# succinctlabs/kzg-rs

Hardware: AMD Instinct MI355X
Metric: blobs/sec verify_blob_kzg_proof_batch (higher is better)
Workload: dtype u32 limbs (255-bit Fr / 381-bit Fp modular integers); 1 GPU; verify_blob_kzg_proof_batch, batches of 1024 synthetic blobs (4096 Fr each), device-resident, known-tau test setup (BASELINE.json configs[1]); one step = one launch group of 256 independent batches = 262144 blobs per GPU; blobs_per_gpu_per_batch=1024, batch=1024, parallelism=shard-by-blob x1, groups_in_flight=4

## Files before the change

kzg_rs_amd/csrc/capi_settings.hpp:

```cpp

#include <atomic>
#include <condition_variable>
#include <deque>
#include <memory>
struct DevProgram {
    SlpProgram p{};
    void* blob = nullptr;
};

struct DevProgram2 {
    Slp2Program p{};
    void* blob = nullptr;
};

constexpr size_t MAX_WORLD = 64;
constexpr size_t LATENCY_PAIRING_MAX = 32;
constexpr size_t MAX_BATCHES_PER_LAUNCH = 16384;
constexpr unsigned MSM_MAX_SLICES = 32;
constexpr size_t SLICED_MAX_BLOBS = 16384;
constexpr size_t LATENCY_MAX_BLOBS = 4096;
struct Workspace {
    size_t cap_n = 0;
    size_t cap_b = 0;
    size_t pending_n = 0, pending_b = 0, finish_b = 0;
// ... 177 lines not shown
    return run_program(s->verify, d_in, s->d_prep, d_out, instances, st);
}

static KzgRet settings_build(KzgSettings* s, const uint8_t tau_g2[96]);
static KzgRet settings_common(KzgSettings** out, const uint8_t tau_g2[96]) {
    int ndev = 0;
    if (hipGetDeviceCount(&ndev) != hipSuccess || ndev == 0) {
        (void)hipGetLastError();
        return fail(KZG_ERROR, "no HIP device: this library has no CPU fallback");
    }
    KzgSettings* s = new KzgSettings();
    KzgRet rc = settings_build(s, tau_g2);
    if (rc != KZG_OK) {
        const std::string msg = g_err;
        kzg_settings_free(s);
        g_err = msg;
        return rc;
    }
    if (opt_flag("coalesce", true)) {
        s->small = new SmallQueue();
        s->small->max_lanes = (size_t)std::max(1L, std::min((long)SMALL_LANES_MAX, opt_int("small_lanes", 2)));
        s->small->lane_two_streams = ab_int("small_streams", 3) == 2;
        s->small->lane_priority = ab_int("small_priority", 1) ? 1 : 0;
        s->small->linger_us = std::max(0L, std::min(2000L, opt_int("small_linger_us", 250)));
        s->small->linger_gap_us = std::max(1L, std::min(1000L, ab_int("small_linger_gap_us", 40)));
        s->small->cap_proofs = (size_t)std::max(1L, std::min(1024L, ab_int("small_cap_proofs", 1024)));
    }
    *out = s;
    return KZG_OK;
}
static KzgRet stream_make(hipStream_t* st, int priority) {
    if (priority) {
        int least = 0, greatest = 0;
        HIPCHK(hipDeviceGetStreamPriorityRange(&least, &greatest));
        HIPCHK(hipStreamCreateWithPriority(st, hipStreamNonBlocking, greatest));
    } else HIPCHK(hipStreamCreateWithFlags(st, hipStreamNonBlocking));
    return KZG_OK;
}
static KzgRet settings_streams(KzgSettings* s, bool single_stream, int priority = 0) {
    HIPCHK(hipGetDevice(&s->device));
    s->stream_priority = priority;
    KzgRet rc_s = stream_make(&s->s_plain[0], priority);
    if (rc_s != KZG_OK) return rc_s;
    s->s1 = s->s_sha = s->s_plain[0];
    HIPCHK(hipDeviceGetAttribute(&s->n_cus, hipDeviceAttributeMultiprocessorCount, s->device));
    if (single_stream) s->s2 = s->s1;
    else {
        if ((rc_s = stream_make(&s->s_plain[1], priority)) != KZG_OK) return rc_s;
        s->s2 = s->s_plain[1];
    }
    for (auto& e : s->ev) HIPCHK(hipEventCreate(&e));
    return KZG_OK;
}
static KzgRet settings_lane(KzgSettings** out, const KzgSettings* parent, int priority = 0) {
    KzgSettings* l = new KzgSettings();
    l->borrowed = true;
    l->d_M = parent->d_M; l->d_DM = parent->d_DM; l->d_M29 = parent->d_M29; l->d_DM29 = parent->d_DM29;
    l->d_eval_a = parent->d_eval_a; l->d_eval_b = parent->d_eval_b; l->d_eval_c = parent->d_eval_c;
    l->d_tau4 = parent->d_tau4; l->d_prep = parent->d_prep; l->d_prep29 = parent->d_prep29;
    l->d_gen_mult = parent->d_gen_mult; l->d_gen_mult_aff = parent->d_gen_mult_aff;
    l->prep = parent->prep; l->verify = parent->verify; l->verify2 = parent->verify2;
    l->scalars = parent->scalars; l->verify3 = parent->verify3; l->d_fixed_base = parent->d_fixed_base;
    memcpy(l->tau_g2_bytes, parent->tau_g2_bytes, 96);
    KzgRet rc = settings_streams(l, !parent->s_plain[1], priority);
    if (rc != KZG_OK) {
        const std::string msg = g_err;
        kzg_settings_free(l);
        g_err = msg;
        return rc;
    }
    *out = l;
    return KZG_OK;
}
static KzgRet settings_build(KzgSettings* s, const uint8_t tau_g2[96]) {
    memcpy(s->tau_g2_bytes, tau_g2, 96);
    KzgRet rc_streams = settings_streams(s, opt_flag("single_stream", false));
    if (rc_streams != KZG_OK) return rc_streams;
    HIPCHK(hipMalloc(&s->d_M, sizeof(Fr) * FE_PER_BLOB));
    HIPCHK(hipMalloc(&s->d_DM, sizeof(Fr) * FE_PER_BLOB));
    HIPCHK(hipMalloc(&s->d_M29, sizeof(Fr29Mem) * FE_PER_BLOB));
    HIPCHK(hipMalloc(&s->d_DM29, sizeof(Fr29Mem) * FE_PER_BLOB));
    hipLaunchKernelGGL(k_roots_tables, dim3(FE_PER_BLOB / 64), dim3(64), 0, s->s1, s->d_M, s->d_DM);
    hipLaunchKernelGGL(k_roots_tables29, dim3(FE_PER_BLOB / 64), dim3(64), 0, s->s1, s->d_M, s->d_M29, s->d_DM29);
    HIPCHK(hipMalloc(&s->d_eval_a, sizeof(uint4) * EVAL_SLOTS * 64));
    HIPCHK(hipMalloc(&s->d_eval_b, sizeof(uint4) * EVAL_SLOTS * 64));
    HIPCHK(hipMalloc(&s->d_eval_c, 4 * EVAL_SLOTS * 64));
    hipLaunchKernelGGL(k_eval_tables, dim3(EVAL_SLOTS), dim3(64), 0, s->s1, s->d_M29, s->d_DM29, s->d_eval_a, s->d_eval_b, s->d_eval_c);
    HIPCHK(hipGetLastError());
    KzgRet rc;
    if ((rc = upload_program(s->prep, kzg_slp_prep_begin, kzg_slp_prep_end)) != KZG_OK) return rc;
    if ((rc = upload_program(s->verify, kzg_slp_verify_begin, kzg_slp_verify_end)) != KZG_OK) return rc;
    if ((rc = upload_program2(s->verify2, kzg_slp_verify2_begin, kzg_slp_verify2_end)) != KZG_OK) return rc;
    if ((rc = upload_program2(s->scalars, kzg_slp_scalars_begin, kzg_slp_scalars_end)) != KZG_OK) return rc;
    if ((rc = upload_program2(s->verify3, kzg_slp_verify3_begin, kzg_slp_verify3_end)) != KZG_OK) return rc;
    if ((size_t)(kzg_fixed_base_end - kzg_fixed_base_begin) != FB_TABLE_BYTES) return fail(KZG_ERROR, "embedded fixed-base table has the wrong size");
    HIPCHK(hipMalloc(&s->d_fixed_base, FB_TABLE_BYTES));
    HIPCHK(hipMemcpy(s->d_fixed_base, kzg_fixed_base_begin, FB_TABLE_BYTES, hipMemcpyHostToDevice));
    DevTmp t_bytes, t_flag, t_q;
    HIPCHK(hipMalloc(&t_bytes.p, 96));
    HIPCHK(hipMalloc(&t_flag.p, 4));
    HIPCHK(hipMalloc(&t_q.p, sizeof(Fp) * 8));
    uint8_t* d_bytes = t_bytes.as<uint8_t>();
    uint32_t* d_flag = t_flag.as<uint32_t>();
    Fp* d_q = t_q.as<Fp>();
    HIPCHK(hipMalloc(&s->d_tau4, sizeof(Fp) * 4));
    HIPCHK(hipMalloc(&s->d_prep, sizeof(Fp) * 2 * s->prep.p.n_out));
    HIPCHK(hipMemcpyAsync(d_bytes, tau_g2, 96, hipMemcpyHostToDevice, s->s1));
    hipLaunchKernelGGL(k_g2_decompress, dim3(1), dim3(64), 0, s->s1, d_bytes, d_q, d_flag);
    hipLaunchKernelGGL(k_g2_generator, dim3(1), dim3(64), 0, s->s1, d_q + 4);
    HIPCHK(hipGetLastError());
    uint32_t flag = 0;
    HIPCHK(hipMemcpyAsync(&flag, d_flag, 4, hipMemcpyDeviceToHost, s->s1));
    HIPCHK(hipMemcpyAsync(s->d_tau4, d_q, sizeof(Fp) * 4, hipMemcpyDeviceToDevice, s->s1));
    if ((rc = run_program(s->prep, d_q, nullptr, s->d_prep, 2, s->s1)) != KZG_OK) return rc;
    {
        const int np = (int)(2 * s->prep.p.n_out);
        HIPCHK(hipMalloc(&s->d_prep29, (size_t)64 * np));
        hipLaunchKernelGGL(k_fp_to_fp29mem, dim3((unsigned)((np + 63) / 64)), dim3(64), 0, s->s1, s->d_prep, s->d_prep29, np);
        HIPCHK(hipGetLastError());
    }
    {
        DevTmp t_g, t_gf, t_gm;
        HIPCHK(hipMalloc(&t_g.p, sizeof(G1Aff)));
        HIPCHK(hipMalloc(&t_gf.p, 4));
        constexpr int NG = MSM_CHUNKS + MSM_CHUNKS_LATENCY;
        HIPCHK(hipMalloc(&t_gm.p, sizeof(G1Jac) * NG));
        G1Aff* d_g = t_g.as<G1Aff>();
        uint32_t* d_gf = t_gf.as<uint32_t>();
        G1Jac* d_gm = t_gm.as<G1Jac>();
        hipLaunchKernelGGL(k_set_generator, dim3(1), dim3(64), 0, s->s1, d_g, d_gf, 0);
        hipLaunchKernelGGL(k_g1_multiples, dim3(1), dim3(64), 0, s->s1, d_g, d_gf, d_gm, 1, 1, MSM_CHUNKS);
        hipLaunchKernelGGL(k_g1_multiples, dim3(1), dim3(64), 0, s->s1, d_g, d_gf, d_gm + MSM_CHUNKS, 1, 1, MSM_CHUNKS_LATENCY);
        HIPCHK(hipMalloc(&s->d_gen_mult, sizeof(G1Jac29Mem) * NG));
        hipLaunchKernelGGL(k_jac_to_jac29, dim3(1), dim3(64), 0, s->s1, d_gm, (G1Jac29Mem*)s->d_gen_mult, NG);
        HIPCHK(hipMalloc(&s->d_gen_mult_aff, sizeof(G1Aff29Mem) * MSM_CHUNKS));
        hipLaunchKernelGGL(k_jac29_to_aff29, dim3(1), dim3(64), 0, s->s1, (const G1Jac29Mem*)s->d_gen_mult, s->d_gen_mult_aff, MSM_CHUNKS);
        HIPCHK(hipGetLastError());
        HIPCHK(hipStreamSynchronize(s->s1));
    }
    HIPCHK(hipStreamSynchronize(s->s1));
    if (flag != G1_OK) return fail(KZG_BAD_SETUP, "g2_points[1] is not a valid (finite) compressed G2 point");
    if (s->verify.p.n_set != 2 * s->prep.p.n_out || s->verify.p.n_in != 6 || s->prep.p.n_in != 4 || s->verify2.p.n_set != s->verify.p.n_set ||
        s->verify2.p.n_in != 6 || s->verify2.p.n_out != s->verify.p.n_out)
        return fail(KZG_ERROR, "embedded SLP programs do not fit together");
    if (s->scalars.p.n_in != (uint32_t)SCALARS_INPUTS || s->scalars.p.n_set != 0 || !s->scalars.p.out_values || s->scalars.p.n_out + 6 != (uint32_t)VERIFY3_INPUTS ||
        s->verify3.p.n_in != (uint32_t)VERIFY3_INPUTS || s->verify3.p.n_set != s->verify.p.n_set || s->verify3.p.n_out != (uint32_t)VERIFY3_OUTPUTS || s->verify3.p.out_values)
        return fail(KZG_ERROR, "embedded one-proof programs do not fit together");
    return KZG_OK;
}

static KzgRet settings_load_points(KzgSettings* s, const std::vector<uint8_t>& g1b, const std::vector<uint8_t>& g2b, int N, size_t n2) {
    DevTmp t_bytes, t_flag2, t_gflag, t_tmp;
    HIPCHK(hipMalloc(&t_bytes.p, std::max(g1b.size(), g2b.size())));
    HIPCHK(hipMalloc(&t_flag2.p, 4 * (size_t)N));
    HIPCHK(hipMalloc(&t_tmp.p, sizeof(G1Aff) * (size_t)N));
    uint8_t* d_bytes = t_bytes.as<uint8_t>();
    uint32_t* d_flag2 = t_flag2.as<uint32_t>();
    G1Aff* d_tmp = t_tmp.as<G1Aff>();
    HIPCHK(hipMalloc(&s->d_g1, sizeof(G1Aff) * (size_t)N));
    HIPCHK(hipMalloc(&s->d_g1_flag, 4 * (size_t)N));
    HIPCHK(hipMalloc(&s->d_g1_mult, MULT_ENTRY_BYTES * MSM_CHUNKS * (size_t)N));
    HIPCHK(hipMemcpyAsync(d_bytes, g1b.data(), g1b.size(), hipMemcpyHostToDevice, s->s1));
    hipLaunchKernelGGL(k_g1_decode, dim3((unsigned)((N + 63) / 64)), dim3(64), 0, s->s1, d_bytes, d_bytes, N, s->d_g1, s->d_g1_flag, N, 0);
    hipLaunchKernelGGL((k_g1_decode_multiples29<MSM_CHUNKS, false>), dim3((unsigned)((N + 63) / 64)), dim3(64), 64 * PARK_UINT4_PER_THREAD * sizeof(uint4), s->s1, d_bytes, d_bytes, N, d_tmp,
                       d_flag2, s->d_g1_mult, (G1Jac29Mem*)nullptr, N, N);
    HIPCHK(hipGetLastError());
    s->n_g1 = N;
    DevTmp t_jtmp, t_aff_pts;
    if (msm_affine_enabled()) {
        HIPCHK(hipMalloc(&s->d_g1_mult_aff, sizeof(G1Aff29Mem) * MSM_CHUNKS * (size_t)N));
// ... 193 lines not shown
```

kzg_rs_amd/csrc/capi_verify.hpp:

```cpp

static KzgRet launch_evaluate(const KzgSettings* s, const void* d_blobs, const Fr* d_z, Fr* d_y, uint32_t* d_status, size_t T, bool alone = false,
                              bool stamp = false) {
    unsigned long long* const kt = stamp && s->ws.d_ktime ? s->ws.d_ktime + 4 : nullptr;
    if (T > s->eval_scratch_cap) {
        if (s->d_eval_scratch) HIPCHK(hipFree(s->d_eval_scratch));
        s->d_eval_scratch = nullptr;
        s->eval_scratch_cap = 0;
        const size_t cap = T < 1024 ? 1024 : T;
        HIPCHK(hipMalloc(&s->d_eval_scratch, 4 * (size_t)EVAL_SCRATCH_WORDS * cap));
        s->eval_scratch_cap = cap;
    }
    const unsigned per_lane = (unsigned)((T + 63) / 64);
    hipLaunchKernelGGL(k_eval_powers, dim3(per_lane), dim3(64), 0, s->s1, d_z, s->d_eval_scratch, (int)T);
    const unsigned eval_blocks = (unsigned)((T + EVAL_BLOBS_PER_BLOCK - 1) / EVAL_BLOBS_PER_BLOCK);
    static const long pad_opt = ab_int("eval_lds_pad", -1);
    const size_t lds_pad = pad_opt >= 0 ? (size_t)std::min(120L * 1024, pad_opt) : alone ? 0 : 16384;
    size_t spread_lds = eval_blocks <= (unsigned)s->n_cus ? (size_t)EVAL_SPREAD_LDS : lds_pad;
    if (spread_lds && DYN_LDS(k_blob_evaluate_t<true>, spread_lds) != hipSuccess) {
        (void)hipGetLastError();
        spread_lds = 0;
    }
    hipLaunchKernelGGL(k_blob_evaluate_t<true>, dim3(eval_blocks), dim3(64 * EVAL_BLOBS_PER_BLOCK), spread_lds, s->s1,
                       (const uint8_t*)d_blobs, EvalTables{s->d_eval_a, s->d_eval_b, s->d_eval_c}, s->d_eval_scratch, d_status, (int)T, kt);
    hipLaunchKernelGGL(k_eval_finish, dim3(per_lane), dim3(64), 0, s->s1, s->d_eval_scratch, d_y, (int)T);
    return KZG_OK;
}

static KzgRet launch_challenge(const KzgSettings* s, const void* d_blobs, const void* d_commitments, Fr* d_z, size_t T, hipStream_t st = nullptr) {
    if (!st) st = s->s1;
    static const int forced = opt_is("challenge_kernel", "lane") ? 1 : opt_is("challenge_kernel", "split") ? 2 : opt_is("challenge_kernel", "split2") ? 3 : 0;
    const uint8_t *bl = (const uint8_t*)d_blobs, *cm = (const uint8_t*)d_commitments;
    const int form = forced ? forced : T <= 16384 ? 3 : T <= 49152 ? 2 : 1;
    s->ws.ktime_valid = false;
    if (form == 1) {
        unsigned long long* kt = s->ws.d_ktime;
        if (kt) {
            HIPCHK(hipMemsetAsync(kt, 0, 32, st));
            s->ws.ktime_valid = true;
        }
        hipLaunchKernelGGL(k_blob_challenge_t<4>, dim3((unsigned)((T + 255) / 256)), dim3(256), 0, st, bl, cm, d_z, (int)T, kt);
    } else if (form == 2) {
        hipLaunchKernelGGL(k_blob_challenge_split, dim3((unsigned)((T + 63) / 64)), dim3(128), 0, st, bl, cm, d_z, (int)T);
    } else {
        hipLaunchKernelGGL(k_blob_challenge_split2_t<false>, dim3((unsigned)((T + 63) / 64)), dim3(192), 0, st, bl, cm, d_z, (int)T, 0, 1024, (uint32_t*)nullptr);
    }
    HIPCHK(hipGetLastError());
    return KZG_OK;
}

enum { STAGE_NONE = 0, STAGE_BLOBS = 1, STAGE_CP = 2 };
static KzgRet ws_reserve(const KzgSettings* s, size_t T, size_t B, int stage) {
    Workspace& w = s->ws;
    if (T > w.cap_n || B > w.cap_b) {
        size_t keep_stage = w.cap_stage, keep_cp = w.cap_stage_cp, keep_h = w.cap_hstage;
        uint8_t *sb = w.d_stage_blobs, *sc = w.d_stage_cp, *h0 = w.d_hstage[0], *h1 = w.d_hstage[1];
        w.d_stage_blobs = nullptr;
        w.d_stage_cp = nullptr;
        w.d_hstage[0] = w.d_hstage[1] = nullptr;
        size_t capT = T > w.cap_n ? T : w.cap_n, capB = B > w.cap_b ? B : w.cap_b;
        ws_free(w);
        w.d_stage_blobs = sb;
        w.d_stage_cp = sc;
        w.cap_stage = keep_stage;
        w.cap_stage_cp = keep_cp;
        w.d_hstage[0] = h0;
        w.d_hstage[1] = h1;
        w.cap_hstage = keep_h;
        if (capT < 16) capT = 16;
        const size_t np = 2 * capT + 1;
        const size_t nsc = 2 * capT + capB;
        const size_t nterm = 4 * capT + 2 * capB;
        HIPCHK(hipMalloc(&w.d_z, sizeof(Fr) * capT));
        HIPCHK(hipMalloc(&w.d_y, sizeof(Fr) * capT));
        HIPCHK(hipMalloc(&w.d_scalars, sizeof(Fr) * nsc));
        HIPCHK(hipMalloc(&w.d_partial, sizeof(Fr) * ((capT + 255) / 256 + capB)));
        HIPCHK(hipMalloc(&w.d_r, sizeof(Fr) * capB));
        HIPCHK(hipMalloc(&w.d_status, 4 * capT));
        HIPCHK(hipMalloc(&w.d_pflag, 4 * np));
        HIPCHK(hipMalloc(&w.d_term_point, 4 * nterm));
        HIPCHK(hipMalloc(&w.d_term_scalar, 4 * nterm));
        HIPCHK(hipMalloc(&w.d_sorted, 4 * MSM_WINDOWS * nterm));
        HIPCHK(hipMalloc(&w.d_points, sizeof(G1Aff) * np));
        HIPCHK(hipMalloc(&w.d_window, sizeof(G1Jac) * 2 * MSM_WINDOWS * capB));
        HIPCHK(hipMalloc(&w.d_window_sl, sizeof(G1Jac) * 2 * MSM_WINDOWS * MSM_MAX_SLICES * 4));
        HIPCHK(hipMalloc(&w.d_mult, MULT_ENTRY_BYTES * std::max((size_t)MSM_CHUNKS * np, (size_t)MSM_CHUNKS_LATENCY * std::min(np, (size_t)(2 * LATENCY_MAX_BLOBS + 1)))));
        HIPCHK(hipMalloc(&w.d_ab, sizeof(G1Jac) * 2 * capB));
        HIPCHK(hipMalloc(&w.d_ktime, 128));
        if (msm_affine_enabled()) HIPCHK(hipMalloc(&w.d_jtmp, sizeof(G1Jac29Mem) * np));
        HIPCHK(hipMalloc(&w.d_parts, sizeof(G1Jac) * 2 * capB * MAX_WORLD));
        HIPCHK(hipMalloc(&w.d_send, sizeof(G1Jac) * 2 * MAX_WORLD));
        HIPCHK(hipMalloc(&w.d_slp_in, sizeof(Fp) * 6 * capB));
        HIPCHK(hipMalloc(&w.d_slp_out, sizeof(Fp) * 6 * capB));
        HIPCHK(hipMalloc(&w.d_bytes, 96 * np));
        HIPCHK(hipMalloc(&w.d_records, 160 * capT));
        HIPCHK(hipMalloc(&w.d_sha_mid, 32 * std::min(capT, (size_t)SLICED_MAX_BLOBS)));
        w.off_r = 256 * capT + 4096;
        w.off_part = w.off_r + 32 * capB;
        w.off_out = w.off_part + 288 * capB;
        w.off_parts = w.off_out + 288 * capB;
        w.h_cap = w.off_parts + 288 * capB * MAX_WORLD;
        HIPCHK(hipHostMalloc(&w.h_buf, w.h_cap));
        w.cap_n = capT;
        w.cap_b = capB;
    }
    if (stage != STAGE_NONE && T > w.cap_stage_cp) {
// ... 1250 lines not shown
```

kzg_rs_amd/csrc/fr_kernels.hpp:

```cpp
#pragma once
#include "field.hpp"
#include "fr29.hpp"
#include "sha256.hpp"

namespace kzg {

constexpr int FE_PER_BLOB = 4096;
constexpr int BLOB_BYTES = 131072;

__device__ __forceinline__ uint32_t bitrev12(uint32_t i) { return __brev(i) >> 20; }

__global__ void k_roots_tables(Fr* __restrict__ M, Fr* __restrict__ DM) {
    int j = blockIdx.x * blockDim.x + threadIdx.x;
    if (j >= FE_PER_BLOB) return;
    uint32_t e = bitrev12(j);
    Fr w, acc = FrF::one();
#pragma unroll
    for (int i = 0; i < 8; i++) w.l[i] = consts::FR_OMEGA_MONT[i];
    for (int b = 11; b >= 0; b--) {
        acc = FrF::sqr(acc);
        if ((e >> b) & 1) acc = FrF::mul(acc, w);
    }
    M[j] = acc;
    Fr r2;
// ... 261 lines not shown
        uint32_t* my_mid = SEG ? mid + 8 * (size_t)(live ? i : n - 1) + (a_lane ? 0 : 4) : nullptr;
        if (SEG && M0 > 0) {
            const uint4 q = *reinterpret_cast<const uint4*>(my_mid);
            H0 = q.x; H1 = q.y; H2 = q.z; H3 = q.w;
        }
        __syncthreads();
#pragma unroll 1
        for (int b = 0; b < NBLK; b++) {
            const uint4* src = tile + (b & 1) * (16 * 64) + blob_in_block;
            constexpr int stride = 64;
            uint32_t kw[65];
#pragma unroll
            for (int t = 0; t < 16; t++) {
                const uint4 q = src[t * stride];
                kw[4 * t] = q.x; kw[4 * t + 1] = q.y; kw[4 * t + 2] = q.z; kw[4 * t + 3] = q.w;
            }
            kw[64] = 0;
            Sha2LaneRing r;
            r.x0 = H0; r.x1 = H1; r.x2 = H2; r.dd = H3;
            r.hk = a_lane ? 0u : H3 + kw[0];
            asm volatile("" : "=v"(r.nx));
#pragma unroll
            for (int t = 0; t < 6; t++) sha256_rounds10_2lane(r, kw + 10 * t + 1, c);
            sha256_rounds4_2lane(r, kw + 61, c);
            H0 += r.x0;
            H1 += r.x1;
            H2 += r.x2;
            H3 += a_lane ? r.dd : r.hk;
            __syncthreads();
        }
        if (SEG && !last_seg) {
            if (live) *reinterpret_cast<uint4*>(my_mid) = make_uint4(H0, H1, H2, H3);
            return;
        }
        const uint32_t e0 = (uint32_t)__builtin_amdgcn_update_dpp(0, (int)H0, 0x104, 0xF, 0xF, true), e1 = (uint32_t)__builtin_amdgcn_update_dpp(0, (int)H1, 0x104, 0xF, 0xF, true);
        const uint32_t e2 = (uint32_t)__builtin_amdgcn_update_dpp(0, (int)H2, 0x104, 0xF, 0xF, true), e3 = (uint32_t)__builtin_amdgcn_update_dpp(0, (int)H3, 0x104, 0xF, 0xF, true);
        if (live && a_lane) {
            const uint32_t hh[8] = {H0, H1, H2, H3, e0, e1, e2, e3};
            Fr dgst;
#pragma unroll
            for (int k = 0; k < 8; k++) dgst.l[k] = hh[7 - k];
            z_out[i] = FrF::from_mont(FrF::to_mont(dgst));
        }
    }
}

__device__ __forceinline__ Fr fr_shfl_xor(const Fr& a, int mask) {
    Fr r;
#pragma unroll
    for (int i = 0; i < 8; i++) r.l[i] = __shfl_xor((int)a.l[i], mask, 64);
    return r;
}

struct alignas(16) Fr29Mem {
    uint32_t l[12];
};
__device__ __forceinline__ Fr29 fr29_load(const Fr29Mem* p) {
    const uint4 a = *reinterpret_cast<const uint4*>(p->l), b = *reinterpret_cast<const uint4*>(p->l + 4);
    Fr29 r;
    r.l[0] = a.x; r.l[1] = a.y; r.l[2] = a.z; r.l[3] = a.w;
    r.l[4] = b.x; r.l[5] = b.y; r.l[6] = b.z; r.l[7] = b.w;
    r.l[8] = p->l[8];
    return r;
}
__device__ __forceinline__ Fr29 fr29_shfl_xor(const Fr29& a, int mask) {
    Fr29 r;
#pragma unroll
    for (int i = 0; i < 9; i++) r.l[i] = __shfl_xor((int)a.l[i], mask, 64);
    return r;
}
__global__ void k_roots_tables29(const Fr* __restrict__ M, Fr29Mem* __restrict__ M29, Fr29Mem* __restrict__ DM29) {
    int j = blockIdx.x * blockDim.x + threadIdx.x;
    if (j >= FE_PER_BLOB) return;
    Fr w = FrF::from_mont(M[j]);
    const Fr29 r2 = fr29_const(c29::FR29_R2);
    Fr29 m = fr29_mul(fr29_from_words(w.l), r2), dm = fr29_mul(m, r2);
#pragma unroll
    for (int i = 0; i < 12; i++) {
        M29[j].l[i] = i < 9 ? m.l[i] : 0u;
        DM29[j].l[i] = i < 9 ? dm.l[i] : 0u;
    }
}

constexpr int EVAL_SLOTS = 69;
struct EvalTables {
    const uint4 *a, *b;
    const uint32_t* c;
};
__global__ void k_eval_tables(const Fr29Mem* __restrict__ M29, const Fr29Mem* __restrict__ DM29, uint4* __restrict__ ta,
                              uint4* __restrict__ tb, uint32_t* __restrict__ tc) {
    const int slot = blockIdx.x, lane = threadIdx.x;
    const Fr29Mem* e;
    if (slot < 32) {
        e = DM29 + 2 * (32 * lane + slot);
    } else if (slot < 63) {
        int L = 1, rel = slot - 32;
        while (rel >= (32 >> L)) { rel -= 32 >> L; L++; }
        const int q = (rel << L) | ((1 << L) - 1);
        e = M29 + (((32 * lane + q) >> (L - 1)) & ~1);
    } else {
        e = M29 + ((lane >> (slot - 63)) & ~1);
    }
    ta[slot * 64 + lane] = make_uint4(e->l[0], e->l[1], e->l[2], e->l[3]);
    tb[slot * 64 + lane] = make_uint4(e->l[4], e->l[5], e->l[6], e->l[7]);
    tc[slot * 64 + lane] = e->l[8];
}
__device__ __forceinline__ Fr29 eval_table_load(const EvalTables& t, int slot, int lane) {
    const uint4 a = t.a[slot * 64 + lane], b = t.b[slot * 64 + lane];
    Fr29 r;
    r.l[0] = a.x; r.l[1] = a.y; r.l[2] = a.z; r.l[3] = a.w;
    r.l[4] = b.x; r.l[5] = b.y; r.l[6] = b.z; r.l[7] = b.w;
    r.l[8] = t.c[slot * 64 + lane];
    return r;
}

struct EvalRsrc {
    __amdgpu_buffer_rsrc_t a, b, c;
};
__device__ __forceinline__ Fr29 eval_table_load(const EvalRsrc& t, int slot, uint32_t lane16, uint32_t lane4) {
    typedef uint32_t u32x4 __attribute__((ext_vector_type(4)));
    const u32x4 a = __builtin_amdgcn_raw_buffer_load_b128(t.a, lane16, slot * 1024, 0);
    const u32x4 b = __builtin_amdgcn_raw_buffer_load_b128(t.b, lane16, slot * 1024, 0);
    Fr29 r;
    r.l[0] = a.x; r.l[1] = a.y; r.l[2] = a.z; r.l[3] = a.w;
    r.l[4] = b.x; r.l[5] = b.y; r.l[6] = b.z; r.l[7] = b.w;
    r.l[8] = __builtin_amdgcn_raw_buffer_load_b32(t.c, lane4, slot * 256, 0);
    return r;
}

constexpr int EVAL_SCRATCH_WORDS = 16 * 9;
__global__ __launch_bounds__(64) void k_eval_powers(const Fr* __restrict__ z_in, uint32_t* __restrict__ scratch, int T) {
    const int b = blockIdx.x * 64 + threadIdx.x;
    if (b >= T) return;
    const Fr zin = z_in[b];
    const Fr29 r2 = fr29_const(c29::FR29_R2);
    Fr29* Z = reinterpret_cast<Fr29*>(scratch + (size_t)b * EVAL_SCRATCH_WORDS);
    Fr29 z = fr29_mul(fr29_from_words(zin.l), r2);
    Z[0] = z;
    Z[13] = fr29_mul(z, r2);
    for (int l = 1; l <= 12; l++) {
        z = fr29_mul(z, z);
        Z[l] = z;
    }
}
__global__ __launch_bounds__(64) void k_eval_finish(const uint32_t* __restrict__ scratch, Fr* __restrict__ y_out, int T) {
    const int b = blockIdx.x * 64 + threadIdx.x;
    if (b >= T) return;
    const Fr29* Z = reinterpret_cast<const Fr29*>(scratch + (size_t)b * EVAL_SCRATCH_WORDS);
    const Fr29 n = Z[14], sm = Z[15];
    const Fr29 x = fr29_mul(sm, Z[12]);
    const Fr29 nw = fr29_sub_biased(fr29_add(fr29_mul(n, Z[0]), sm), x);
    const Fr29 y29 = fr29_mul(nw, fr29_const(c29::FR29_INV4096_PLAIN));
    Fr y;
    fr29_to_words(y.l, y29);
    y_out[b] = FrF::reduce_once(y);
}

constexpr int EVAL_BLOBS_PER_BLOCK = 4;
constexpr int EVAL_SPREAD_LDS = 96 * 1024;
template <bool SPLIT>
__global__ __launch_bounds__(256, 3) void k_blob_evaluate_t(const uint8_t* __restrict__ blobs, const EvalTables tab,
                                                       uint32_t* __restrict__ scratch, uint32_t* __restrict__ status, int T,
                                                       unsigned long long* __restrict__ ktime) {
    static_assert(SPLIT, "k_blob_evaluate_t has one form");
    const int wave = threadIdx.x >> 6, lane = threadIdx.x & 63;
    const int blob_idx = blockIdx.x * EVAL_BLOBS_PER_BLOCK + wave;
    const bool active = blob_idx < T;
    __shared__ Fr29 Zs[EVAL_BLOBS_PER_BLOCK][14];
    __shared__ uint4 stack_as[EVAL_BLOBS_PER_BLOCK][4][64], stack_bs[EVAL_BLOBS_PER_BLOCK][4][64];
    __shared__ uint32_t stack_cs[EVAL_BLOBS_PER_BLOCK][4][64];
    Fr29* Z = Zs[wave];
    uint4 (*stack_a)[64] = stack_as[wave], (*stack_b)[64] = stack_bs[wave];
    uint32_t (*stack_c)[64] = stack_cs[wave];
    if (!active) return;
    kstamp_in(ktime);
    const int blob_u = __builtin_amdgcn_readfirstlane(blob_idx);
    uint32_t* const my = scratch + (size_t)blob_u * EVAL_SCRATCH_WORDS;
    for (int i = lane; i < 14 * 9; i += 64) reinterpret_cast<uint32_t*>(Z)[i] = my[i];
    const Fr29 zd = Z[13];
    bool bad = false;
    Fr29 n, psum;
#pragma unroll
    for (int i = 0; i < 9; i++) psum.l[i] = 0;
    uint4 cur[8];
    const __amdgpu_buffer_rsrc_t rs_blob = __builtin_amdgcn_make_buffer_rsrc(const_cast<uint8_t*>(blobs) + (size_t)blob_u * BLOB_BYTES, 0, BLOB_BYTES, 0x00020000);
    EvalRsrc rs;
    rs.a = __builtin_amdgcn_make_buffer_rsrc(const_cast<uint4*>(tab.a), 0, EVAL_SLOTS * 64 * 16, 0x00020000);
    rs.b = __builtin_amdgcn_make_buffer_rsrc(const_cast<uint4*>(tab.b), 0, EVAL_SLOTS * 64 * 16, 0x00020000);
    rs.c = __builtin_amdgcn_make_buffer_rsrc(const_cast<uint32_t*>(tab.c), 0, EVAL_SLOTS * 64 * 4, 0x00020000);
    const uint32_t lane2k = (uint32_t)lane * 2048u, lane16 = (uint32_t)lane * 16u, lane4 = (uint32_t)lane * 4u;
    auto blob_load = [&](int byte_off) {
        typedef uint32_t u32x4 __attribute__((ext_vector_type(4)));
        const u32x4 v = __builtin_amdgcn_raw_buffer_load_b128(rs_blob, lane2k, byte_off, 0);
        return make_uint4(v.x, v.y, v.z, v.w);
    };
#pragma unroll
    for (int i = 0; i < 8; i++) cur[i] = blob_load(16 * i);
    Fr29 leaf0 = eval_table_load(rs, 0, lane16, lane4), leaf1 = eval_table_load(rs, 1, lane16, lane4);
    struct PairOps {
        Fr29 s, u;
    };
    auto convert = [&](const uint4& a_hi, const uint4& a_lo, const uint4& b_hi, const uint4& b_lo) {
        Fr wa = fr_from_be_words(a_hi, a_lo), wb = fr_from_be_words(b_hi, b_lo);
        if (__any((wa.l[7] >= consts::FR_MOD[7]) | (wb.l[7] >= consts::FR_MOD[7]))) bad |= FrF::geq_mod(wa) | FrF::geq_mod(wb);
        const Fr29 pa = fr29_from_words(wa.l), pb = fr29_from_words(wb.l);
        PairOps o;
        o.s = fr29_add(pa, pb);
        o.u = fr29_sub_biased4(pa, pb);
        psum = fr29_add(psum, o.s);
        return o;
    };
    for (int j = 0; j < 16; j++) {
        const int jn = j < 15 ? j + 1 : 15;
        const PairOps p0 = convert(cur[0], cur[1], cur[2], cur[3]);
        __builtin_amdgcn_sched_barrier(0x7);
#pragma unroll
        for (int i = 0; i < 4; i++) cur[i] = blob_load(128 * jn + 16 * i);
        __builtin_amdgcn_sched_barrier(0x7);
        const Fr29 n0 = fr29_mul2(p0.s, zd, p0.u, leaf0);
        const PairOps p1 = convert(cur[4], cur[5], cur[6], cur[7]);
        __builtin_amdgcn_sched_barrier(0x7);
#pragma unroll
        for (int i = 4; i < 8; i++) cur[i] = blob_load(128 * jn + 16 * i);
        Fr29 root = eval_table_load(rs, 32 + j, lane16, lane4);
        __builtin_amdgcn_sched_barrier(0x7);
        const Fr29 n1 = fr29_mul2(p1.s, zd, p1.u, leaf1);
        psum = fr29_normalize(psum);
        __builtin_amdgcn_sched_barrier(0x7);
        leaf0 = eval_table_load(rs, 2 * jn, lane16, lane4);
        leaf1 = eval_table_load(rs, 2 * jn + 1, lane16, lane4);
        Fr29 root_next = eval_table_load(rs, 48 + (j >> 1), lane16, lane4);
        __builtin_amdgcn_sched_barrier(0x7);
        n = fr29_mul2(fr29_add(n0, n1), Z[1], fr29_sub_biased4(n0, n1), root);
        root = root_next;
        int level = 2;
        for (int jj = j; jj & 1; jj >>= 1) {
            Fr29 na;
            const uint4 h0 = stack_a[level - 2][lane], h1 = stack_b[level - 2][lane];
            na.l[0] = h0.x; na.l[1] = h0.y; na.l[2] = h0.z; na.l[3] = h0.w;
            na.l[4] = h1.x; na.l[5] = h1.y; na.l[6] = h1.z; na.l[7] = h1.w;
            na.l[8] = stack_c[level - 2][lane];
            root_next = eval_table_load(rs, 64 - (32 >> level) + (j >> level), lane16, lane4);
            const Fr29 sum = fr29_add(na, n), dif = fr29_sub_biased4(na, n);
            n = fr29_mul2(sum, Z[level], dif, root);
            root = root_next;
            level++;
        }
        if (j != 15) {
            stack_a[level - 2][lane] = make_uint4(n.l[0], n.l[1], n.l[2], n.l[3]);
            stack_b[level - 2][lane] = make_uint4(n.l[4], n.l[5], n.l[6], n.l[7]);
            stack_c[level - 2][lane] = n.l[8];
        }
    }
    for (int L = 6; L < 12; L++) {
        int sh = L - 6;
        Fr29 other = fr29_shfl_xor(n, 1 << sh);
        bool left = ((lane >> sh) & 1) == 0;
        Fr29 na, nb;
#pragma unroll
        for (int i = 0; i < 9; i++) {
            na.l[i] = left ? n.l[i] : other.l[i];
            nb.l[i] = left ? other.l[i] : n.l[i];
        }
        const Fr29 sum = fr29_add(na, nb), dif = fr29_sub_biased4(na, nb);
        n = fr29_mul2(sum, Z[L], dif, eval_table_load(tab, 63 + sh, lane));
    }
    Fr29 sm = fr29_mul(psum, fr29_const(c29::FR29_R2));
    for (int sh = 1; sh < 64; sh <<= 1) {
        sm = fr29_add(sm, fr29_shfl_xor(sm, sh));
        if (sh & 0x2A) sm = fr29_normalize(sm);
    }
    unsigned long long any_bad = __ballot(bad);
    sm = fr29_mul(sm, fr29_const(c29::FR29_ONE));
    if (lane < 9) {
        uint32_t vn = n.l[0], vs = sm.l[0];
#pragma unroll
        for (int i = 1; i < 9; i++) {
            vn = lane == i ? n.l[i] : vn;
            vs = lane == i ? sm.l[i] : vs;
        }
        my[14 * 9 + lane] = vn;
        my[15 * 9 + lane] = vs;
    }
    if (lane == 0 && any_bad) atomicOr(&status[blob_u], 1u);
    kstamp_out(ktime);
}

__device__ __forceinline__ Fr fr_shfl(const Fr& a, int src) {
    Fr r;
#pragma unroll
    for (int i = 0; i < 8; i++) r.l[i] = __shfl((int)a.l[i], src, 64);
    return r;
}
__device__ inline Fr fr_inverse_mont(const Fr& a) {
    return pow_limbs<Fr, 8>(a, consts::FR_R_MINUS_2, FrF::one(), [](const Fr& x, const Fr& y) { return FrF::mul(x, y); });
}
__global__ __launch_bounds__(64) void k_blob_quotient(const uint8_t* __restrict__ blobs, const Fr* __restrict__ z_in,
                                                      const Fr* __restrict__ y_in, const Fr* __restrict__ M, Fr* __restrict__ out,
                                                      uint32_t* __restrict__ status) {
    const int b = blockIdx.x, lane = threadIdx.x;
    const Fr zM = FrF::to_mont(z_in[b]), y = y_in[b];
    const uint4* src = reinterpret_cast<const uint4*>(blobs + (size_t)b * BLOB_BYTES) + (size_t)lane * 128;
    Fr* o = out + (size_t)b * FE_PER_BLOB + 64 * lane;
    const Fr* Ml = M + 64 * lane;
    Fr acc = FrF::one();
    int special = -1;
    for (int k = 0; k < 64; k++) {
        Fr d = FrF::sub(Ml[k], zM);
        if (FrF::is_zero(d)) {
            special = k;
            d = FrF::one();
        }
        o[k] = acc;
        acc = FrF::mul(acc, d);
    }
    Fr incl = acc;
    for (int sh = 1; sh < 64; sh <<= 1) {
        Fr up = fr_shfl(incl, lane >= sh ? lane - sh : lane);
        if (lane >= sh) incl = FrF::mul(incl, up);
    }
    const Fr total = fr_shfl(incl, 63);
    Fr excl = fr_shfl(incl, lane ? lane - 1 : 0);
    if (lane == 0) excl = FrF::one();
    const Fr inv_total = fr_inverse_mont(total);
    Fr sfx = acc;
    for (int sh = 1; sh < 64; sh <<= 1) {
        Fr dn = fr_shfl(sfx, lane + sh < 64 ? lane + sh : lane);
        if (lane + sh < 64) sfx = FrF::mul(sfx, dn);
    }
    Fr sfx_excl = fr_shfl(sfx, lane < 63 ? lane + 1 : 63);
    if (lane == 63) sfx_excl = FrF::one();
    Fr running = FrF::mul(inv_total, sfx_excl);
    bool bad = false;
    Fr wsum = FrF::zero();
    for (int k = 63; k >= 0; k--) {
        Fr d = FrF::sub(Ml[k], zM);
        if (k == special) d = FrF::one();
        const Fr inv_d = FrF::mul(running, FrF::mul(excl, o[k]));
        running = FrF::mul(running, d);
        const Fr p = fr_from_be_words(src[2 * k], src[2 * k + 1]);
        bad |= FrF::geq_mod(p);
        Fr q = FrF::mul(FrF::sub(p, y), inv_d);
        if (k == special) q = FrF::zero();
        o[k] = q;
        wsum = FrF::add(wsum, FrF::mul(q, Ml[k]));
    }
    const unsigned long long any_special = __ballot(special >= 0);
    if (any_special) {
        for (int sh = 1; sh < 64; sh <<= 1) wsum = FrF::add(wsum, fr_shfl_xor(wsum, sh));
        if (special >= 0) o[special] = FrF::neg(FrF::mul(wsum, fr_inverse_mont(zM)));
    }
    if (__ballot(bad) && lane == 0) atomicOr(&status[b], 1u);
}

}
```

Before: 4.788 million blobs/s.

## Evaluate two blobs per wave with 32 lanes per blob in blob evaluation

Generalizes the barycentric blob-evaluation kernel to a configurable lanes-per-blob geometry and sets it to 32, so each 64-lane wave processes two blobs with twice the elements per lane. This shrinks the root tables, the LDS stack per blob and the cross-lane butterfly tail, which now uses ds_bpermute instead of shuffle plus select. It also lowers the default LDS padding used to limit occupancy. The trade is longer serial per-lane loops and more register pressure, in exchange for fewer shuffle stages and less table and LDS traffic per blob.

```diff
diff --git a/kzg_rs_amd/csrc/capi_settings.hpp b/kzg_rs_amd/csrc/capi_settings.hpp
--- a/kzg_rs_amd/csrc/capi_settings.hpp
+++ b/kzg_rs_amd/csrc/capi_settings.hpp
@@ -283,10 +283,10 @@
     HIPCHK(hipMalloc(&s->d_DM29, sizeof(Fr29Mem) * FE_PER_BLOB));
     hipLaunchKernelGGL(k_roots_tables, dim3(FE_PER_BLOB / 64), dim3(64), 0, s->s1, s->d_M, s->d_DM);
     hipLaunchKernelGGL(k_roots_tables29, dim3(FE_PER_BLOB / 64), dim3(64), 0, s->s1, s->d_M, s->d_M29, s->d_DM29);
-    HIPCHK(hipMalloc(&s->d_eval_a, sizeof(uint4) * EVAL_SLOTS * 64));
-    HIPCHK(hipMalloc(&s->d_eval_b, sizeof(uint4) * EVAL_SLOTS * 64));
-    HIPCHK(hipMalloc(&s->d_eval_c, 4 * EVAL_SLOTS * 64));
-    hipLaunchKernelGGL(k_eval_tables, dim3(EVAL_SLOTS), dim3(64), 0, s->s1, s->d_M29, s->d_DM29, s->d_eval_a, s->d_eval_b, s->d_eval_c);
+    HIPCHK(hipMalloc(&s->d_eval_a, sizeof(uint4) * EVAL_SLOTS * EVAL_LPB));
+    HIPCHK(hipMalloc(&s->d_eval_b, sizeof(uint4) * EVAL_SLOTS * EVAL_LPB));
+    HIPCHK(hipMalloc(&s->d_eval_c, 4 * EVAL_SLOTS * EVAL_LPB));
+    hipLaunchKernelGGL(k_eval_tables, dim3(EVAL_SLOTS), dim3(EVAL_LPB), 0, s->s1, s->d_M29, s->d_DM29, s->d_eval_a, s->d_eval_b, s->d_eval_c);
     HIPCHK(hipGetLastError());
     KzgRet rc;
     if ((rc = upload_program(s->prep, kzg_slp_prep_begin, kzg_slp_prep_end)) != KZG_OK) return rc;
diff --git a/kzg_rs_amd/csrc/capi_verify.hpp b/kzg_rs_amd/csrc/capi_verify.hpp
--- a/kzg_rs_amd/csrc/capi_verify.hpp
+++ b/kzg_rs_amd/csrc/capi_verify.hpp
@@ -14,13 +14,13 @@
     hipLaunchKernelGGL(k_eval_powers, dim3(per_lane), dim3(64), 0, s->s1, d_z, s->d_eval_scratch, (int)T);
     const unsigned eval_blocks = (unsigned)((T + EVAL_BLOBS_PER_BLOCK - 1) / EVAL_BLOBS_PER_BLOCK);
     static const long pad_opt = ab_int("eval_lds_pad", -1);
-    const size_t lds_pad = pad_opt >= 0 ? (size_t)std::min(120L * 1024, pad_opt) : alone ? 0 : 16384;
+    const size_t lds_pad = pad_opt >= 0 ? (size_t)std::min(120L * 1024, pad_opt) : alone ? 0 : 5120;
     size_t spread_lds = eval_blocks <= (unsigned)s->n_cus ? (size_t)EVAL_SPREAD_LDS : lds_pad;
     if (spread_lds && DYN_LDS(k_blob_evaluate_t<true>, spread_lds) != hipSuccess) {
         (void)hipGetLastError();
         spread_lds = 0;
     }
-    hipLaunchKernelGGL(k_blob_evaluate_t<true>, dim3(eval_blocks), dim3(64 * EVAL_BLOBS_PER_BLOCK), spread_lds, s->s1,
+    hipLaunchKernelGGL(k_blob_evaluate_t<true>, dim3(eval_blocks), dim3(64 * EVAL_WAVES_PER_BLOCK), spread_lds, s->s1,
                        (const uint8_t*)d_blobs, EvalTables{s->d_eval_a, s->d_eval_b, s->d_eval_c}, s->d_eval_scratch, d_status, (int)T, kt);
     hipLaunchKernelGGL(k_eval_finish, dim3(per_lane), dim3(64), 0, s->s1, s->d_eval_scratch, d_y, (int)T);
     return KZG_OK;
diff --git a/kzg_rs_amd/csrc/fr_kernels.hpp b/kzg_rs_amd/csrc/fr_kernels.hpp
--- a/kzg_rs_amd/csrc/fr_kernels.hpp
+++ b/kzg_rs_amd/csrc/fr_kernels.hpp
@@ -367,49 +367,57 @@
     }
 }
 
-constexpr int EVAL_SLOTS = 69;
+template <int LPB>
+struct EvalGeom {
+    static_assert(LPB == 64 || LPB == 32 || LPB == 16, "lanes per blob: 64, 32 or 16 (8 lanes: the tail needs 9 lanes per blob, the stack 64 KB of LDS)");
+    static constexpr int BPW = 64 / LPB;
+    static constexpr int E = FE_PER_BLOB / LPB;
+    static constexpr int P = E / 2;
+    static constexpr int NIT = E / 4;
+    static constexpr int XL = LPB == 64 ? 6 : LPB == 32 ? 5 : 4;
+    static constexpr int LL = 11 - XL;
+    static constexpr int STACK = LL - 1;
+    static constexpr int SLOTS = 2 * P - 1 + XL;
+};
+constexpr int EVAL_LPB = 32;
+
+constexpr int EVAL_SLOTS = EvalGeom<EVAL_LPB>::SLOTS;
 struct EvalTables {
     const uint4 *a, *b;
     const uint32_t* c;
 };
 __global__ void k_eval_tables(const Fr29Mem* __restrict__ M29, const Fr29Mem* __restrict__ DM29, uint4* __restrict__ ta,
                               uint4* __restrict__ tb, uint32_t* __restrict__ tc) {
-    const int slot = blockIdx.x, lane = threadIdx.x;
+    using G = EvalGeom<EVAL_LPB>;
+    const int slot = blockIdx.x, t = threadIdx.x;
     const Fr29Mem* e;
-    if (slot < 32) {
-        e = DM29 + 2 * (32 * lane + slot);
-    } else if (slot < 63) {
-        int L = 1, rel = slot - 32;
-        while (rel >= (32 >> L)) { rel -= 32 >> L; L++; }
+    if (slot < G::P) {
+        e = DM29 + 2 * (G::P * t + slot);
+    } else if (slot < 2 * G::P - 1) {
+        int L = 1, rel = slot - G::P;
+        while (rel >= (G::P >> L)) { rel -= G::P >> L; L++; }
         const int q = (rel << L) | ((1 << L) - 1);
-        e = M29 + (((32 * lane + q) >> (L - 1)) & ~1);
+        e = M29 + (((G::P * t + q) >> (L - 1)) & ~1);
     } else {
-        e = M29 + ((lane >> (slot - 63)) & ~1);
-    }
-    ta[slot * 64 + lane] = make_uint4(e->l[0], e->l[1], e->l[2], e->l[3]);
-    tb[slot * 64 + lane] = make_uint4(e->l[4], e->l[5], e->l[6], e->l[7]);
-    tc[slot * 64 + lane] = e->l[8];
-}
-__device__ __forceinline__ Fr29 eval_table_load(const EvalTables& t, int slot, int lane) {
-    const uint4 a = t.a[slot * 64 + lane], b = t.b[slot * 64 + lane];
+        e = M29 + ((t >> (slot - (2 * G::P - 1))) & ~1);
+    }
+    ta[slot * EVAL_LPB + t] = make_uint4(e->l[0], e->l[1], e->l[2], e->l[3]);
+    tb[slot * EVAL_LPB + t] = make_uint4(e->l[4], e->l[5], e->l[6], e->l[7]);
+    tc[slot * EVAL_LPB + t] = e->l[8];
+}
+
+struct EvalRsrc {
+    __amdgpu_buffer_rsrc_t a, b, c;
+};
+template <int LPB>
+__device__ __forceinline__ Fr29 eval_table_load(const EvalRsrc& t, int slot, uint32_t lane16, uint32_t lane4) {
+    typedef uint32_t u32x4 __attribute__((ext_vector_type(4)));
+    const u32x4 a = __builtin_amdgcn_raw_buffer_load_b128(t.a, lane16, slot * (16 * LPB), 0);
+    const u32x4 b = __builtin_amdgcn_raw_buffer_load_b128(t.b, lane16, slot * (16 * LPB), 0);
     Fr29 r;
     r.l[0] = a.x; r.l[1] = a.y; r.l[2] = a.z; r.l[3] = a.w;
     r.l[4] = b.x; r.l[5] = b.y; r.l[6] = b.z; r.l[7] = b.w;
-    r.l[8] = t.c[slot * 64 + lane];
-    return r;
-}
-
-struct EvalRsrc {
-    __amdgpu_buffer_rsrc_t a, b, c;
-};
-__device__ __forceinline__ Fr29 eval_table_load(const EvalRsrc& t, int slot, uint32_t lane16, uint32_t lane4) {
-    typedef uint32_t u32x4 __attribute__((ext_vector_type(4)));
-    const u32x4 a = __builtin_amdgcn_raw_buffer_load_b128(t.a, lane16, slot * 1024, 0);
-    const u32x4 b = __builtin_amdgcn_raw_buffer_load_b128(t.b, lane16, slot * 1024, 0);
-    Fr29 r;
-    r.l[0] = a.x; r.l[1] = a.y; r.l[2] = a.z; r.l[3] = a.w;
-    r.l[4] = b.x; r.l[5] = b.y; r.l[6] = b.z; r.l[7] = b.w;
-    r.l[8] = __builtin_amdgcn_raw_buffer_load_b32(t.c, lane4, slot * 256, 0);
+    r.l[8] = __builtin_amdgcn_raw_buffer_load_b32(t.c, lane4, slot * (4 * LPB), 0);
     return r;
 }
 
@@ -441,47 +449,53 @@
     y_out[b] = FrF::reduce_once(y);
 }
 
-constexpr int EVAL_BLOBS_PER_BLOCK = 4;
+constexpr int EVAL_WAVES_PER_BLOCK = 4;
+constexpr int EVAL_BLOBS_PER_BLOCK = EVAL_WAVES_PER_BLOCK * EvalGeom<EVAL_LPB>::BPW;
 constexpr int EVAL_SPREAD_LDS = 96 * 1024;
 template <bool SPLIT>
 __global__ __launch_bounds__(256, 3) void k_blob_evaluate_t(const uint8_t* __restrict__ blobs, const EvalTables tab,
                                                        uint32_t* __restrict__ scratch, uint32_t* __restrict__ status, int T,
                                                        unsigned long long* __restrict__ ktime) {
     static_assert(SPLIT, "k_blob_evaluate_t has one form");
+    constexpr int LPB = EVAL_LPB;
+    using G = EvalGeom<LPB>;
     const int wave = threadIdx.x >> 6, lane = threadIdx.x & 63;
-    const int blob_idx = blockIdx.x * EVAL_BLOBS_PER_BLOCK + wave;
-    const bool active = blob_idx < T;
-    __shared__ Fr29 Zs[EVAL_BLOBS_PER_BLOCK][14];
-    __shared__ uint4 stack_as[EVAL_BLOBS_PER_BLOCK][4][64], stack_bs[EVAL_BLOBS_PER_BLOCK][4][64];
-    __shared__ uint32_t stack_cs[EVAL_BLOBS_PER_BLOCK][4][64];
-    Fr29* Z = Zs[wave];
+    const int sub = lane / LPB, t = lane % LPB;
+    const int first_blob = (blockIdx.x * EVAL_WAVES_PER_BLOCK + wave) * G::BPW;
+    __shared__ Fr29 Zs[EVAL_WAVES_PER_BLOCK][G::BPW][14];
+    __shared__ uint4 stack_as[EVAL_WAVES_PER_BLOCK][G::STACK][64], stack_bs[EVAL_WAVES_PER_BLOCK][G::STACK][64];
+    __shared__ uint32_t stack_cs[EVAL_WAVES_PER_BLOCK][G::STACK][64];
+    Fr29* Z = Zs[wave][sub];
     uint4 (*stack_a)[64] = stack_as[wave], (*stack_b)[64] = stack_bs[wave];
     uint32_t (*stack_c)[64] = stack_cs[wave];
-    if (!active) return;
+    if (first_blob >= T) return;
     kstamp_in(ktime);
-    const int blob_u = __builtin_amdgcn_readfirstlane(blob_idx);
-    uint32_t* const my = scratch + (size_t)blob_u * EVAL_SCRATCH_WORDS;
-    for (int i = lane; i < 14 * 9; i += 64) reinterpret_cast<uint32_t*>(Z)[i] = my[i];
+    const int blob_u = __builtin_amdgcn_readfirstlane(first_blob);
+    const int blobs_here = T - blob_u < G::BPW ? T - blob_u : G::BPW;
+    const __amdgpu_buffer_rsrc_t rs_my = __builtin_amdgcn_make_buffer_rsrc(scratch + (size_t)blob_u * EVAL_SCRATCH_WORDS, 0, blobs_here * EVAL_SCRATCH_WORDS * 4, 0x00020000);
+    for (int i = t; i < 14 * 9; i += LPB)
+        reinterpret_cast<uint32_t*>(Z)[i] = __builtin_amdgcn_raw_buffer_load_b32(rs_my, (uint32_t)(sub * EVAL_SCRATCH_WORDS + i) * 4u, 0, 0);
     const Fr29 zd = Z[13];
     bool bad = false;
     Fr29 n, psum;
 #pragma unroll
     for (int i = 0; i < 9; i++) psum.l[i] = 0;
     uint4 cur[8];
-    const __amdgpu_buffer_rsrc_t rs_blob = __builtin_amdgcn_make_buffer_rsrc(const_cast<uint8_t*>(blobs) + (size_t)blob_u * BLOB_BYTES, 0, BLOB_BYTES, 0x00020000);
+    const __amdgpu_buffer_rsrc_t rs_blob = __builtin_amdgcn_make_buffer_rsrc(const_cast<uint8_t*>(blobs) + (size_t)blob_u * BLOB_BYTES, 0, blobs_here * BLOB_BYTES, 0x00020000);
     EvalRsrc rs;
-    rs.a = __builtin_amdgcn_make_buffer_rsrc(const_cast<uint4*>(tab.a), 0, EVAL_SLOTS * 64 * 16, 0x00020000);
-    rs.b = __builtin_amdgcn_make_buffer_rsrc(const_cast<uint4*>(tab.b), 0, EVAL_SLOTS * 64 * 16, 0x00020000);
-    rs.c = __builtin_amdgcn_make_buffer_rsrc(const_cast<uint32_t*>(tab.c), 0, EVAL_SLOTS * 64 * 4, 0x00020000);
-    const uint32_t lane2k = (uint32_t)lane * 2048u, lane16 = (uint32_t)lane * 16u, lane4 = (uint32_t)lane * 4u;
+    rs.a = __builtin_amdgcn_make_buffer_rsrc(const_cast<uint4*>(tab.a), 0, G::SLOTS * LPB * 16, 0x00020000);
+    rs.b = __builtin_amdgcn_make_buffer_rsrc(const_cast<uint4*>(tab.b), 0, G::SLOTS * LPB * 16, 0x00020000);
+    rs.c = __builtin_amdgcn_make_buffer_rsrc(const_cast<uint32_t*>(tab.c), 0, G::SLOTS * LPB * 4, 0x00020000);
+    const uint32_t lane_off = (uint32_t)lane * (32u * G::E), lane16 = (uint32_t)t * 16u, lane4 = (uint32_t)t * 4u;
     auto blob_load = [&](int byte_off) {
         typedef uint32_t u32x4 __attribute__((ext_vector_type(4)));
-        const u32x4 v = __builtin_amdgcn_raw_buffer_load_b128(rs_blob, lane2k, byte_off, 0);
+        const u32x4 v = __builtin_amdgcn_raw_buffer_load_b128(rs_blob, lane_off, byte_off, 0);
         return make_uint4(v.x, v.y, v.z, v.w);
     };
+    auto table = [&](int slot) { return eval_table_load<LPB>(rs, slot, lane16, lane4); };
 #pragma unroll
     for (int i = 0; i < 8; i++) cur[i] = blob_load(16 * i);
-    Fr29 leaf0 = eval_table_load(rs, 0, lane16, lane4), leaf1 = eval_table_load(rs, 1, lane16, lane4);
+    Fr29 leaf0 = table(0), leaf1 = table(1);
     struct PairOps {
         Fr29 s, u;
     };
@@ -495,8 +509,8 @@
         psum = fr29_add(psum, o.s);
         return o;
     };
-    for (int j = 0; j < 16; j++) {
-        const int jn = j < 15 ? j + 1 : 15;
+    for (int j = 0; j < G::NIT; j++) {
+        const int jn = j < G::NIT - 1 ? j + 1 : G::NIT - 1;
         const PairOps p0 = convert(cur[0], cur[1], cur[2], cur[3]);
         __builtin_amdgcn_sched_barrier(0x7);
 #pragma unroll
@@ -507,14 +521,14 @@
         __builtin_amdgcn_sched_barrier(0x7);
 #pragma unroll
         for (int i = 4; i < 8; i++) cur[i] = blob_load(128 * jn + 16 * i);
-        Fr29 root = eval_table_load(rs, 32 + j, lane16, lane4);
+        Fr29 root = table(G::P + j);
         __builtin_amdgcn_sched_barrier(0x7);
         const Fr29 n1 = fr29_mul2(p1.s, zd, p1.u, leaf1);
         psum = fr29_normalize(psum);
         __builtin_amdgcn_sched_barrier(0x7);
-        leaf0 = eval_table_load(rs, 2 * jn, lane16, lane4);
-        leaf1 = eval_table_load(rs, 2 * jn + 1, lane16, lane4);
-        Fr29 root_next = eval_table_load(rs, 48 + (j >> 1), lane16, lane4);
+        leaf0 = table(2 * jn);
+        leaf1 = table(2 * jn + 1);
+        Fr29 root_next = table(G::P + G::P / 2 + (j >> 1));
         __builtin_amdgcn_sched_barrier(0x7);
         n = fr29_mul2(fr29_add(n0, n1), Z[1], fr29_sub_biased4(n0, n1), root);
         root = root_next;
@@ -525,49 +539,49 @@
             na.l[0] = h0.x; na.l[1] = h0.y; na.l[2] = h0.z; na.l[3] = h0.w;
             na.l[4] = h1.x; na.l[5] = h1.y; na.l[6] = h1.z; na.l[7] = h1.w;
             na.l[8] = stack_c[level - 2][lane];
-            root_next = eval_table_load(rs, 64 - (32 >> level) + (j >> level), lane16, lane4);
+            root_next = table(2 * G::P - (G::P >> level) + (j >> level));
             const Fr29 sum = fr29_add(na, n), dif = fr29_sub_biased4(na, n);
             n = fr29_mul2(sum, Z[level], dif, root);
             root = root_next;
             level++;
         }
-        if (j != 15) {
+        if (j != G::NIT - 1) {
             stack_a[level - 2][lane] = make_uint4(n.l[0], n.l[1], n.l[2], n.l[3]);
             stack_b[level - 2][lane] = make_uint4(n.l[4], n.l[5], n.l[6], n.l[7]);
             stack_c[level - 2][lane] = n.l[8];
         }
     }
-    for (int L = 6; L < 12; L++) {
-        int sh = L - 6;
-        Fr29 other = fr29_shfl_xor(n, 1 << sh);
-        bool left = ((lane >> sh) & 1) == 0;
+    for (int L = G::LL + 1; L < 12; L++) {
+        const int sh = L - G::LL - 1;
+        const int src_l = (lane & ~(1 << sh)) << 2, src_r = (lane | (1 << sh)) << 2;
         Fr29 na, nb;
 #pragma unroll
         for (int i = 0; i < 9; i++) {
-            na.l[i] = left ? n.l[i] : other.l[i];
-            nb.l[i] = left ? other.l[i] : n.l[i];
+            na.l[i] = (uint32_t)__builtin_amdgcn_ds_bpermute(src_l, (int)n.l[i]);
+            nb.l[i] = (uint32_t)__builtin_amdgcn_ds_bpermute(src_r, (int)n.l[i]);
         }
         const Fr29 sum = fr29_add(na, nb), dif = fr29_sub_biased4(na, nb);
-        n = fr29_mul2(sum, Z[L], dif, eval_table_load(tab, 63 + sh, lane));
+        n = fr29_mul2(sum, Z[L], dif, table(2 * G::P - 1 + sh));
     }
     Fr29 sm = fr29_mul(psum, fr29_const(c29::FR29_R2));
-    for (int sh = 1; sh < 64; sh <<= 1) {
+    for (int sh = 1; sh < LPB; sh <<= 1) {
         sm = fr29_add(sm, fr29_shfl_xor(sm, sh));
         if (sh & 0x2A) sm = fr29_normalize(sm);
     }
-    unsigned long long any_bad = __ballot(bad);
+    const unsigned long long any_bad = (__ballot(bad) >> (lane - t)) & (~0ull >> (64 - LPB));
     sm = fr29_mul(sm, fr29_const(c29::FR29_ONE));
-    if (lane < 9) {
+    if (t < 9) {
         uint32_t vn = n.l[0], vs = sm.l[0];
 #pragma unroll
         for (int i = 1; i < 9; i++) {
-            vn = lane == i ? n.l[i] : vn;
-            vs = lane == i ? sm.l[i] : vs;
-        }
-        my[14 * 9 + lane] = vn;
-        my[15 * 9 + lane] = vs;
-    }
-    if (lane == 0 && any_bad) atomicOr(&status[blob_u], 1u);
+            vn = t == i ? n.l[i] : vn;
+            vs = t == i ? sm.l[i] : vs;
+        }
+        const uint32_t mine = (uint32_t)(sub * EVAL_SCRATCH_WORDS + t) * 4u;
+        __builtin_amdgcn_raw_buffer_store_b32(vn, rs_my, mine, 14 * 9 * 4, 0);
+        __builtin_amdgcn_raw_buffer_store_b32(vs, rs_my, mine, 15 * 9 * 4, 0);
+    }
+    if (t == 0 && sub < blobs_here && any_bad) atomicOr(&status[blob_u + sub], 1u);
     kstamp_out(ktime);
 }
 
```

Measured after the change: 4.826 million blobs/s (median of 6 runs). About the same (+0.8%).
